# onolab-tmu/overiva

Measured on AMD Instinct MI355X. Metric: AuxIVA iterations/sec (2048 bins x 4000 frames x 8 mics), higher is better.
Workload: dtype f32

## Files before the change

overiva_amd/csrc/kernel_choice.h:

```cpp
#pragma once
#include <algorithm>
#include <functional>

#include "overiva_hip.h"

namespace oiva {

inline int ceil_div(int a, int b) { return (a + b - 1) / b; }
inline int round_up(int a, int b) { return (a + b - 1) / b * b; }

constexpr int kNarrowMax = 16;
constexpr int kWideMax = OIVA_MAX_CHANNELS;

constexpr int kBinsPerWave = 16;
constexpr int kPhasesPerWave = 4;
constexpr int kBlock = 256;
constexpr int kWaves = kBlock / 64;

enum class CovKind { Lane, Pair32, Pair64, Quad, Half16, Hmfma, Half16F64, Hmfma64, Mfma, Wide };
enum class PowKind { Lane, Mfma, Lds, Wide };
constexpr int kCovKinds = 10, kPowKinds = 4;
static_assert((int)CovKind::Wide + 1 == kCovKinds && (int)PowKind::Wide + 1 == kPowKinds, "one traits row per kind");

struct CovGeom {
// ... 74 lines not shown
    Partials partials;
    int launches;
    bool padded_x;
    bool quad_switch;
    bool fusable;
    bool update_arith;
    CovKind unit;
};
constexpr CovTraits kCovTraits[kCovKinds] = {
     {[](int M, int K) { return M >= 1 && M <= 8 && K >= 1 && K <= M; }, nullptr, kBinsPerWave, 16, Partials::F64, 1, false, false, true, false, CovKind::Lane},
     {[](int M, int K) { return M == 8 && K >= 3; }, [](int) { return 4; }, 32, 8, Partials::F64, 2, false, false, false, true, CovKind::Pair32},
     {[](int M, int) { return M == 8; }, [](int K) { return K >= 2 ? 2 : 1; }, 32, 8, Partials::F64, 2, false, false, false, false, CovKind::Pair64},
     {[](int M, int K) { return M >= 10 && M <= 16 && M % 2 == 0 && K >= 1 && K <= 4; }, [](int K) { return K >= 2 ? 2 : 1; }, kBinsPerWave, 8, Partials::F64, 2, true, true, false, true, CovKind::Quad},
     {[](int M, int K) { return M >= 10 && M <= 16 && M % 2 == 0 && K >= 1 && K <= 16; }, [](int K) { return K <= 8 ? 8 : (K <= 12 ? 12 : 16); }, 2, 16, Partials::F64, 2, true, true, false, true, CovKind::Half16},
     {[](int M, int K) { return M >= 10 && M <= 16 && M % 2 == 0 && K >= 9 && K <= 16; }, [](int K) { return K <= 8 ? 8 : (K <= 12 ? 12 : 16); }, 2, 32, Partials::F32IfPart32, 2, true, true, false, true, CovKind::Half16},
     {[](int M, int K) { return M >= 10 && M <= 16 && M % 2 == 0 && K >= 3 && K <= 16; }, [](int K) { return K <= 4 ? 4 : 8; }, 2, 16, Partials::F64, 2, true, true, false, true, CovKind::Mfma},
     {[](int M, int K) { return M == 16 && K >= 9 && K <= 16; }, [](int K) { return K <= 4 ? 4 : 8; }, 2, 32, Partials::F64, 2, true, true, false, true, CovKind::Mfma},
     {[](int M, int K) { return M >= 9 && M <= 16 && K >= 1 && K <= M; }, [](int) { return 1; }, kBinsPerWave, 4, Partials::Acc, 2, false, false, false, true, CovKind::Mfma},
     {[](int M, int K) { return M > kNarrowMax && M <= kWideMax && K >= 1 && K <= M; }, [](int K) { return std::min(K, 2); }, 1, 4, Partials::F64, 2, false, false, false, true, CovKind::Wide},
};
constexpr const CovTraits& traits(CovKind k) { return kCovTraits[(int)k]; }
constexpr bool partials_f64(const CovGeom& g, bool cov_f64) {
    return traits(g.kind).partials == Partials::F64 || (traits(g.kind).partials == Partials::Acc ? cov_f64 : !g.part32);
}

struct PowTraits {
    bool (*supported)(int M, int K);
    int (*sources)(int K);
    int bins;
    int quantum;
    bool padded_x;
    bool occupancy;
};
constexpr int pow_sources_per_pass(int , int K) {
    return K >= 3 ? 4 : (K >= 2 ? 2 : 1);
}
constexpr PowTraits kPowTraits[kPowKinds] = {
     {[](int M, int K) { return M >= 1 && M <= kNarrowMax && K >= 1 && K <= M && (M <= 8 || K <= 4); }, [](int K) { return pow_sources_per_pass(0, K); }, kBinsPerWave * kWaves, 4, false, true},
     {[](int M, int K) { return M > 8 && M <= kNarrowMax && K > 4 && K <= M; }, [](int K) { return pow_sources_per_pass(0, K); }, kBinsPerWave * kWaves, 4, true, false},
     {[](int M, int K) { return M == 16 && K > 4 && K <= M; }, [](int K) { return pow_sources_per_pass(0, K); }, kBinsPerWave * kWaves, 4, false, false},
     {[](int M, int K) { return M > kNarrowMax && M <= kWideMax && K >= 1 && K <= M; }, [](int K) { return K >= 3 ? 4 : K; }, kBinsPerWave * kWaves, 4, false, false},
};
constexpr const PowTraits& traits(PowKind k) { return kPowTraits[(int)k]; }

struct ChoiceIn {
    int T, F, F_total, M, K;
    int n_cu;
    bool cov_f64, upd_f64;
    bool cov_quad_on = true;
    bool cov_hmfma_on = true;
    bool part32 = false;
    bool kc_wide = true;
    bool power_lds = true;
};
struct Occupancy {
    std::function<int(int M, int kc, bool f64)> cov_blocks_per_cu;
    std::function<int(int M, int kp, int tcp)> pow_blocks_per_cu;
};

inline int lane_sources_per_pass(int M, int K, bool f64, bool short_axis, bool kc_wide) {
    const int regs = M * M * (f64 ? 2 : 1);
    int kc = 1;
    if (K >= 2 && regs * 2 <= 144) kc = 2;
    if (K >= 3 && regs * 4 <= 144) kc = 4;
    if (!f64 && kc_wide) {
        if (M == 7 && (K == 3 || K == 5 || K == 6 || (K == 7 && short_axis))) kc = 3;
        if (M == 5 && K >= 5) kc = 5;
    }
    return kc;
}

inline int pick_splits(int capacity, int blocks_per_split, int T, int min_frames) {
    int ns = std::max(1, capacity / std::max(1, blocks_per_split));
    ns = std::min(ns, std::max(1, T / std::max(1, min_frames)));
    return ns;
}

inline int mixed_min_splits(int capacity, int blocks_per_split, int T) {
    if (T >= 1024) return 8;
    const int one_round = std::max(1, capacity / std::max(1, blocks_per_split));
    return std::max(1, std::min(std::min(4, one_round), T / 16));
}

constexpr bool padded_channels(int M) { return M > 8 && M <= kNarrowMax && M % 2 == 1; }

inline CovKind choose_cov_kind(const ChoiceIn& c) {
    const int M = c.M, K = c.K;
    if (M > kNarrowMax) return CovKind::Wide;
    if (M <= 8) {
        if (!c.cov_f64 && traits(CovKind::Pair32).supported(M, K)) return CovKind::Pair32;
        if (c.cov_f64 && traits(CovKind::Pair64).supported(M, K)) return CovKind::Pair64;
        return CovKind::Lane;
    }
    const int Mc = M + (padded_channels(M) ? 1 : 0);
    if (!c.cov_f64 && c.cov_quad_on && traits(CovKind::Quad).supported(Mc, K) && (K <= 2 || c.upd_f64)) return CovKind::Quad;
    if (c.cov_quad_on && (c.cov_f64 ? traits(CovKind::Half16F64).supported(Mc, K) : K > 4 && traits(CovKind::Half16).supported(Mc, K))) {
        const CovKind hm = c.cov_f64 ? CovKind::Hmfma64 : CovKind::Hmfma;
        if (c.cov_hmfma_on && traits(hm).supported(Mc, K)) return hm;
        return c.cov_f64 ? CovKind::Half16F64 : CovKind::Half16;
    }
    return CovKind::Mfma;
}

inline CovGeom choose_cov(const ChoiceIn& c, const Occupancy& occ, int nsplit_req) {
    CovGeom g{};
    g.kind = choose_cov_kind(c);
// ... 18 lines not shown
                if (c.upd_f64) nsplit = std::max(nsplit, mixed_min_splits(n_cu * 2, blocks, T));
            }
            break;
        case CovKind::Half16:
        case CovKind::Hmfma:
        case CovKind::Half16F64:
        case CovKind::Hmfma64: {
            const bool hm = g.kind == CovKind::Hmfma || g.kind == CovKind::Hmfma64;
            if (nsplit <= 0) {
                const int chains = hm ? 8 : 4;
                nsplit = c.cov_f64 ? (!hm && g.kc == 4 && T >= 1024 ? 2 : 1) : ceil_div(T, chains * (c.upd_f64 ? 128 : 256));
                const int per_cu = hm ? (c.cov_f64 ? 2 : 3) : c.cov_f64 && g.kc == 4 ? 4 : 2;
                const int groups = hm ? F : g.nbg * ceil_div(K, g.kc);
                while (groups * nsplit < per_cu * n_cu && ceil_div(T, nsplit + 1) >= 64) ++nsplit;
            }
            if (t.partials == Partials::F32IfPart32) g.part32 = c.part32 ? 1 : 0;
            break;
        }
        case CovKind::Mfma:
            if (nsplit <= 0) {
                nsplit = ceil_div(T, 512);
                const int waves = F * ceil_div(K, 4);
                while (waves * nsplit < 2 * 4 * n_cu && ceil_div(T, nsplit + 1) >= 64) ++nsplit;
            }
            break;
        case CovKind::Lane:
        case CovKind::Pair32:
        case CovKind::Pair64:
            if (nsplit <= 0) {
                const int nz = ceil_div(K, g.kc);
                int bpc = 2;
                if (g.kind == CovKind::Lane && (bpc = occ.cov_blocks_per_cu(c.M, g.kc, c.cov_f64)) < 1) bpc = 2;
                nsplit = pick_splits(n_cu * bpc, g.nbg * nz, T, T >= 1024 ? 128 : 64);
                if (nsplit >= 12 && g.nbg * nz * nsplit >= n_cu * bpc) nsplit = nsplit * 7 / 8;
                const int cap = (g.nbg * nz * 32 >= n_cu) ? 32 : 64;
                nsplit = std::min(nsplit, cap);
                if (g.kind == CovKind::Pair32 && c.upd_f64) {
                    const int by_chain = T >= 1024 ? 8 : std::min(4, ceil_div(T, 256));
                    nsplit = std::max(nsplit, std::min(by_chain, mixed_min_splits(n_cu * bpc, g.nbg * nz, T)));
                }
            }
            break;
    }
    g.tc = round_up(ceil_div(T, nsplit), t.quantum);
    g.nsplit = ceil_div(T, g.tc);
    return g;
}

inline PowKind choose_pow_kind(const ChoiceIn& c) {
    if (c.M > kNarrowMax) return PowKind::Wide;
    if (!traits(PowKind::Mfma).supported(c.M, c.K)) return PowKind::Lane;
    if (c.power_lds && traits(PowKind::Lds).supported(c.M, c.K) && c.F >= kBinsPerWave * kWaves && c.T >= 16) return PowKind::Lds;
    return PowKind::Mfma;
}

inline PowGeom choose_pow(const ChoiceIn& c, const Occupancy& occ, int nsplit_req) {
    PowGeom g{};
    g.kind = choose_pow_kind(c);
    const PowTraits& t = traits(g.kind);
    const int T = c.T, n_cu = c.n_cu;
    g.nb = ceil_div(c.F, t.bins);
    g.kp = t.sources(c.K);
    int nsplit = nsplit_req;
    if (g.kind == PowKind::Wide) {
        const int groups = g.nb * ceil_div(c.K, g.kp);
        if (nsplit <= 0) nsplit = pick_splits(n_cu * 4, groups, T, 16);
        g.tcp = round_up(ceil_div(T, nsplit), t.quantum);
        g.nsplit = ceil_div(T, g.tcp);
        return g;
    }
    if (nsplit <= 0) {
        const int per_cu_x12 = (g.kp == 1 && c.M <= 8) ? 24 : 12;
        nsplit = pick_splits(std::max(n_cu / 2, n_cu * per_cu_x12 / std::max(c.M, 1)), g.nb, T, 32);
    }
    int tcp = round_up(ceil_div(T, nsplit), t.quantum);
    tcp = std::min(std::max(tcp, 4), kPowMaxFrames);
    g.tcp = tcp;
    g.nsplit = ceil_div(T, tcp);
    if (t.occupancy) {
        const int bpc = occ.pow_blocks_per_cu(c.M, g.kp, g.tcp);
        if (bpc > 0) g.rounds = (int)((((long long)g.nb * g.nsplit * ceil_div(c.K, g.kp)) + (long long)bpc * n_cu - 1) / ((long long)bpc * n_cu));
    }
    return g;
}

}
```

overiva_amd/csrc/kernels_cov.hip:

```cpp

#include <cstdint>
#include <cstdlib>

#include "oiva_device.h"
#include "cov_arith.h"

namespace oiva {
namespace {

constexpr int kCovUnroll = 2;
constexpr int kChunk = 16;
constexpr int kLdsStride = kBlock + 1;

template <int M, int KC, typename ACC, typename At>
__device__ __forceinline__ void reduce_and_store_at(At&& at, ACC* lds, double* __restrict__ Vpart, int F, int K, int k0) {
    constexpr int NA = M * M;
    constexpr int NACC = NA * KC;
    const int tid = threadIdx.x;
    const int bb = tid >> 4, aa = tid & 15;
    const int fo = blockIdx.x * kBinsPerWave + bb;
    double* out = Vpart + (((size_t)blockIdx.y * F + fo) * K + k0) * NA;
#pragma unroll
    for (int r0 = 0; r0 < NACC; r0 += kChunk) {
        __syncthreads();
// ... 56 lines not shown
    for (int kk = 0; kk < KC; ++kk)
#pragma unroll
        for (int a = 0; a < NA; ++a) acc[kk][a] = 0;

    const size_t frame_stride = (size_t)F * M;
    const float2* pbase = X + (size_t)fc * M;
    for (int i = 0; i < nsteps; i += kCovUnroll) {
        float xr[kCovUnroll][M], xi[kCovUnroll][M], rv[kCovUnroll][KC];
#pragma unroll
        for (int u = 0; u < kCovUnroll; ++u) {
            const int t = t_begin + q + 16 * (i + u);
            const int tcl = t < t_end ? t : T - 1;
            if constexpr (!UNIT) {
#pragma unroll
                for (int kk = 0; kk < KC; ++kk) {
                    const int k = k0 + kk;
                    rv[u][kk] = R[(size_t)tcl * K + (k < K ? k : K - 1)];
                }
            }
            load_x<M>(pbase + (size_t)tcl * frame_stride, xr[u], xi[u]);
        }
#pragma unroll
        for (int u = 0; u < kCovUnroll; ++u) {
            const int t = t_begin + q + 16 * (i + u);
            const bool live = t < t_end;
            ACC w[KC], ar[M], ai[M];
#pragma unroll
            for (int kk = 0; kk < KC; ++kk) {
                const bool on = live && (UNIT || k0 + kk < K);
                if constexpr (UNIT) {
                    w[kk] = on ? ACC(1) : ACC(0);
                } else if constexpr (sizeof(ACC) == 8) {
                    double rn = (double)rv[u][kk] * ginv[kk];
                    rn = rn < (double)kEpsR ? (double)kEpsR : rn;
                    w[kk] = on ? 1. / rn : 0.;
                } else {
                    w[kk] = on ? activation_weight(rv[u][kk], (float)ginv[kk]) : 0.f;
                }
            }
#pragma unroll
            for (int c = 0; c < M; ++c) {
                ar[c] = (ACC)xr[u][c];
                ai[c] = (ACC)xi[u][c];
            }
            accumulate<M, KC, UNIT, ACC>(acc, ar, ai, w);
        }
    }

    reduce_and_store<M, KC, ACC>(acc, lds, Vpart, F, K, k0);
}

constexpr int kDmaStages = 4;

template <int PIECES>
__device__ __forceinline__ void ring_read(unsigned addr, float4 (&v)[PIECES]);
template <int PIECES>
__device__ __forceinline__ void ring_read_rows(unsigned addr, float4 (&v)[PIECES]);

template <>
__device__ __forceinline__ void ring_read<4>(unsigned addr, float4 (&v)[4]) {
    asm volatile(
        "s_waitcnt vmcnt(12)\n\t"
        "ds_read_b128 %0, %4\n\t"
        "ds_read_b128 %1, %4 offset:1024\n\t"
        "ds_read_b128 %2, %4 offset:2048\n\t"
        "ds_read_b128 %3, %4 offset:3072\n\t"
        "s_waitcnt lgkmcnt(0)"
        : "=&v"(v[0]), "=&v"(v[1]), "=&v"(v[2]), "=&v"(v[3])
        : "v"(addr)
        : "memory");
}
template <>
__device__ __forceinline__ void ring_read<2>(unsigned addr, float4 (&v)[2]) {
    asm volatile(
        "s_waitcnt vmcnt(6)\n\t"
        "ds_read_b128 %0, %2\n\t"
        "ds_read_b128 %1, %2 offset:1024\n\t"
        "s_waitcnt lgkmcnt(0)"
        : "=&v"(v[0]), "=&v"(v[1])
        : "v"(addr)
        : "memory");
}

template <>
__device__ __forceinline__ void ring_read_rows<4>(unsigned addr, float4 (&v)[4]) {
    asm volatile(
        "s_waitcnt vmcnt(12)\n\t"
        "ds_read_b128 %0, %4\n\t"
        "ds_read_b128 %1, %4 offset:16\n\t"
        "ds_read_b128 %2, %4 offset:32\n\t"
        "ds_read_b128 %3, %4 offset:48\n\t"
        "s_waitcnt lgkmcnt(0)"
        : "=&v"(v[0]), "=&v"(v[1]), "=&v"(v[2]), "=&v"(v[3])
        : "v"(addr)
        : "memory");
}
template <>
__device__ __forceinline__ void ring_read_rows<2>(unsigned addr, float4 (&v)[2]) {
    asm volatile(
        "s_waitcnt vmcnt(6)\n\t"
        "ds_read_b128 %0, %2\n\t"
        "ds_read_b128 %1, %2 offset:16\n\t"
        "s_waitcnt lgkmcnt(0)"
        : "=&v"(v[0]), "=&v"(v[1])
        : "v"(addr)
        : "memory");
}

#ifdef OIVA_COVDMA_TRACE
__device__ long long g_cd_trace[8 * 2048];
#define CD_STAMP(slot)                                                                                                            \
    do {                                                                                                                          \
        if (threadIdx.x == 0 && blockIdx.z == 0) g_cd_trace[(blockIdx.y * gridDim.x + blockIdx.x) * 8 + (slot)] = wall_clock64(); \
    } while (0)
#else
#define CD_STAMP(slot) \
    do {               \
    } while (0)
#endif

template <int M, int KC>
__global__ __launch_bounds__(kBlock, 2) void cov_dma_kernel(const float2* __restrict__ X, const float* __restrict__ R,
                                                            float* __restrict__ wscale, int model, int raw,
                                                            double* __restrict__ Vpart, int T, int F, int K, int tc, int xplain) {
    constexpr int NA = M * M;
    constexpr int PIECES = M / 2;
    constexpr int STAGE = PIECES * 64;
    static_assert(M % 2 == 0 && (PIECES == 2 || PIECES == 4), "LDS-DMA path: M in {4, 8}");
    __shared__ float4 ring[kWaves * kDmaStages * STAGE];
    static_assert(sizeof(float4) * kWaves * kDmaStages * STAGE >= sizeof(float) * kChunk * kLdsStride,
                  "reduction scratch aliases the ring");

    const int tid = threadIdx.x;
    const int lane = tid & 63;
    const int wave = __builtin_amdgcn_readfirstlane(tid >> 6);
    const int b = lane & (kBinsPerWave - 1);
    const int ql = lane >> 4;
    const int q = wave * kPhasesPerWave + ql;
    const int f = blockIdx.x * kBinsPerWave + b;
    const int fc = f < F ? f : F - 1;
    const int k0 = blockIdx.z * KC;
    const int t_begin = blockIdx.y * tc;
    const int t_end = min(T, t_begin + tc);
    const int nsteps = (t_end - t_begin + 15) >> 4;

    constexpr bool kPacked = KC == 2;
    float acc[kPacked ? 1 : KC][kPacked ? 1 : NA];
    PkAcc2<M> pacc;
    if constexpr (kPacked) {
        pacc.clear();
    } else {
#pragma unroll
        for (int kk = 0; kk < KC; ++kk)
#pragma unroll
            for (int a = 0; a < NA; ++a) acc[kk][a] = 0.f;
    }

    float ginv[KC];
    float4* wring = ring + wave * kDmaStages * STAGE;
    const unsigned rd_base = (unsigned)(uintptr_t)(wring) + lane * 16;
    const size_t frame_stride = (size_t)F * M;
    const float2* pbase = X + (size_t)fc * M;
    using Rows = XRows<M>;
    const int row_off = Rows::offset(lane, blockIdx.x * kBinsPerWave, F);
    const unsigned rd_rows = (unsigned)(uintptr_t)(wring) + Rows::slot(b, ql) * 16;
    auto plain = [&](int i) { return M != 8 || x_group_plain(kXGroup * i, xplain); };

    auto issue = [&](int i, int s) {
        if (!plain(i)) {
            Rows::issue_nt(X, frame_stride, row_off, lane, t_begin + wave * kPhasesPerWave + 16 * i, i < nsteps ? t_end : 0, T, wring + s * STAGE);
            return;
        }
        const int t = t_begin + q + 16 * i;
        const int tcl = (i < nsteps && t < t_end) ? t : T - 1;
        const float2* src = pbase + (size_t)tcl * frame_stride;
#pragma unroll
        for (int j = 0; j < PIECES; ++j)
            __builtin_amdgcn_global_load_lds((gvoid_t*)(src + 2 * j), (lvoid_t*)(wring + s * STAGE + j * 64), 16, 0, 0);
    };
    const float m0 = ql == 0 ? 1.f : 0.f, m1 = ql == 1 ? 1.f : 0.f, m2 = ql == 2 ? 1.f : 0.f, m3 = ql == 3 ? 1.f : 0.f;
    auto consume = [&](int i, int s) {
        const int tw = min(t_begin + wave * kPhasesPerWave + 16 * i, T);
        const float* rp = R + (size_t)tw * K;
        float w[KC];
#pragma unroll
        for (int kk = 0; kk < KC; ++kk) {
            const int k = k0 + kk < K ? k0 + kk : K - 1;
            const float r = m0 * rp[k] + m1 * rp[K + k] + m2 * rp[2 * K + k] + m3 * rp[3 * K + k];
            const float live = (t_begin + wave * kPhasesPerWave + 16 * i + ql < t_end && k0 + kk < K) ? 1.f : 0.f;
            w[kk] = activation_weight(r, ginv[kk]) * live;
        }
        float4 v[PIECES];
        if (plain(i))
            ring_read<PIECES>(rd_base + s * STAGE * 16, v);
        else
            ring_read_rows<PIECES>(rd_rows + s * STAGE * 16, v);
#if defined(OIVA_COVDMA_ABLATE) && (OIVA_COVDMA_ABLATE & 1)
        if constexpr (kPacked) {
            if (v[0].x == 12345.f) pacc.add(reinterpret_cast<const v2f(&)[M]>(v), v2f{w[0], w[1]});
            return;
        }
#endif
        if constexpr (kPacked) {
            v2f x[M];
#pragma unroll
            for (int j = 0; j < PIECES; ++j) {
                x[2 * j] = v2f{v[j].x, v[j].y};
                x[2 * j + 1] = v2f{v[j].z, v[j].w};
            }
            pacc.add(x, v2f{w[0], w[1]});
        } else {
            float xr[M], xi[M];
#pragma unroll
            for (int j = 0; j < PIECES; ++j) {
                xr[2 * j] = v[j].x;
                xi[2 * j] = v[j].y;
                xr[2 * j + 1] = v[j].z;
                xi[2 * j + 1] = v[j].w;
            }
            accumulate<M, KC, false, float>(acc, xr, xi, w);
        }
    };

    CD_STAMP(0);
    issue(0, 0);
    issue(1, 1);
    issue(2, 2);
#pragma unroll
    for (int kk = 0; kk < KC; ++kk) {
        const int k = k0 + kk;
        ginv[kk] = 1.f;
        if (raw & 1) continue;
#if defined(OIVA_COVDMA_ABLATE) && (OIVA_COVDMA_ABLATE & 4)
        const float gamma = R[k < K ? k : K - 1] + 1.f;
#else
        const float gamma = (float)gamma_of(R, T, K, k < K ? k : K - 1);
#endif
        ginv[kk] = 1.f / gamma;
        if (blockIdx.x == 0 && blockIdx.y == 0 && threadIdx.x == 0 && k < K && wscale != nullptr)
            wscale[k] = model == OIVA_MODEL_LAPLACE ? gamma : sqrtf(gamma);
    }

    CD_STAMP(1);
    int i = 0;
    for (; i + 4 <= nsteps; i += 4) {
        issue(i + 3, 3); consume(i, 0);
        issue(i + 4, 0); consume(i + 1, 1);
        issue(i + 5, 1); consume(i + 2, 2);
        issue(i + 6, 2); consume(i + 3, 3);
// ... 144 lines not shown
```

overiva_amd/csrc/kernels_demix.hip:

```cpp
#include "oiva_device.h"
#include "demix_arith.h"

namespace oiva {
namespace {

constexpr int kPowUnroll = 2;

template <int M, int KP, bool NT = false>
__global__ __launch_bounds__(kBlock) void power_kernel(const float2* __restrict__ X, const float2* __restrict__ What,
                                                       float* __restrict__ Ppart, int T, int F, int K, int tcp, int rev, PowOrder ord,
                                                       int xplain, int xctc) {
    extern __shared__ __attribute__((aligned(16))) float sp[];
    const int tid = threadIdx.x;
    const int lane = tid & 63;
    const int wave = NT ? __builtin_amdgcn_readfirstlane(tid >> 6) : tid >> 6;
    const int b = lane & 15;
    const int q = lane >> 4;
    const int f = (blockIdx.x * kWaves + wave) * kBinsPerWave + b;
    const bool fvalid = f < F;
    const int fc = fvalid ? f : F - 1;
    const int k0 = blockIdx.z * KP;
    const int chunk = ord.cs > 0 ? power_chunk_tail_first(blockIdx.y, gridDim.y, ord) : (int)blockIdx.y;
    const int t_begin = chunk * tcp;
    const int t_end = min(T, t_begin + tcp);
    const int len = t_end - t_begin;
    const int nsteps = (len + 3) >> 2;
    const int ngroups = (nsteps + kPowUnroll - 1) / kPowUnroll;

    float wr[KP][M], wi[KP][M];
    load_wconj<M, KP>(What, fc, k0, K, wr, wi);

    const size_t frame_stride = (size_t)F * M;
    const float2* pbase = X + (size_t)fc * M;
    int off0 = 0, row_off = 0;
    float4* wrows = nullptr;
    if constexpr (NT) {
        __shared__ float4 rows[kWaves * kPowUnroll * 32 * M];
        off0 = t_begin % xctc;
        row_off = XRows<M>::offset(lane, (blockIdx.x * kWaves + wave) * kBinsPerWave, F);
        wrows = rows + wave * kPowUnroll * 32 * M;
    }
    for (int g = 0; g < ngroups; ++g) {
        const int i = (rev ? ngroups - 1 - g : g) * kPowUnroll;
        float xr[kPowUnroll][M], xi[kPowUnroll][M];
        bool plain[kPowUnroll];
#pragma unroll
        for (int u = 0; u < kPowUnroll; ++u) {
            const int tl = 4 * (i + u) + q;
            const int t = tl < len ? t_begin + tl : T - 1;
            plain[u] = !NT || x_group_plain(x_split_offset(off0, 4 * (i + u), xctc), xplain);
            if constexpr (NT) {
                if (!plain[u]) {
                    XRows<M>::issue_nt(X, frame_stride, row_off, lane, t_begin + 4 * (i + u), t_end, T, wrows + u * 32 * M);
                    continue;
                }
            }
            load_x<M>(pbase + (size_t)t * frame_stride, xr[u], xi[u]);
        }
#pragma unroll
        for (int u = 0; u < kPowUnroll; ++u) {
            const int tl = 4 * (i + u) + q;
            const bool live = tl < len;
            if constexpr (NT) {
                if (!plain[u]) {
                    const float4* v = wrows + u * 32 * M + XRows<M>::slot(b, q);
#pragma unroll
                    for (int j = 0; j < M / 2; ++j) {
                        const float4 p = v[j];
                        xr[u][2 * j] = p.x, xi[u][2 * j] = p.y, xr[u][2 * j + 1] = p.z, xi[u][2 * j + 1] = p.w;
                    }
                }
            }
#pragma unroll
            for (int kk = 0; kk < KP; ++kk) {
                float yr, yi;
                demix_one<M>(wr[kk], wi[kk], xr[u], xi[u], yr, yi);
                float pw = fmaf(yr, yr, yi * yi);
                pw = fvalid ? pw : 0.f;
                pw = row16_sum(pw);
                if (b == 0 && live) sp[(wave * tcp + tl) * KP + kk] = pw;
            }
        }
    }
    __syncthreads();
    for (int e = tid; e < len * KP; e += kBlock) {
        const int tl = e / KP, kk = e - tl * KP;
        float s = sp[(0 * tcp + tl) * KP + kk];
#pragma unroll
        for (int w = 1; w < kWaves; ++w) s += sp[(w * tcp + tl) * KP + kk];
        if (k0 + kk < K) Ppart[((size_t)blockIdx.x * T + t_begin + tl) * K + k0 + kk] = s;
    }
}

template <int M, int KP>
__global__ __launch_bounds__(kBlock) void stats_kernel(const float2* __restrict__ X, const float2* __restrict__ What,
                                                       float* __restrict__ Spart, int T, int F, int K, int tc) {
    __shared__ float lds[3 * KP * (kBlock + 1)];
    const int tid = threadIdx.x;
    const int b = tid & 15;
    const int q = tid >> 4;
    const int f = blockIdx.x * kBinsPerWave + b;
    const int fc = f < F ? f : F - 1;
    const int k0 = blockIdx.z * KP;
    const int t_begin = blockIdx.y * tc;
    const int t_end = min(T, t_begin + tc);
    const int nsteps = (t_end - t_begin + 15) >> 4;

    float wr[KP][M], wi[KP][M];
    load_wconj<M, KP>(What, fc, k0, K, wr, wi);
    float nr[KP], ni[KP], dn[KP];
#pragma unroll
    for (int kk = 0; kk < KP; ++kk) nr[kk] = ni[kk] = dn[kk] = 0.f;

    const size_t frame_stride = (size_t)F * M;
    const float2* px = X + ((size_t)(t_begin + q) * F + fc) * M;
    for (int i = 0; i < nsteps; ++i) {
        const int t = t_begin + q + 16 * i;
        if (t < t_end) {
            float xr[M], xi[M];
            load_x<M>(px, xr, xi);
#pragma unroll
            for (int kk = 0; kk < KP; ++kk) {
                float yr, yi;
                demix_one<M>(wr[kk], wi[kk], xr, xi, yr, yi);
                nr[kk] = fmaf(xr[0], yr, fmaf(xi[0], yi, nr[kk]));
                ni[kk] = fmaf(xr[0], yi, fmaf(-xi[0], yr, ni[kk]));
                dn[kk] = fmaf(yr, yr, fmaf(yi, yi, dn[kk]));
            }
        }
        px += 16 * frame_stride;
    }
#pragma unroll
    for (int kk = 0; kk < KP; ++kk) {
// ... 175 lines not shown
```

overiva_amd/csrc/oiva_device.h:

```cpp
#pragma once
#include "oiva_internal.h"

#include <type_traits>
#include <utility>

namespace oiva {

constexpr float kEpsR = 1e-15f;

__device__ __forceinline__ double block_sum(double v, double* scratch) {
#pragma unroll
    for (int off = 32; off > 0; off >>= 1) v += __shfl_xor(v, off, 64);
    const int wave = threadIdx.x >> 6;
    __syncthreads();
    if ((threadIdx.x & 63) == 0) scratch[wave] = v;
    __syncthreads();
    double s = 0.;
#pragma unroll
    for (int w = 0; w < kWaves; ++w) s += scratch[w];
    return s;
}

__device__ __forceinline__ double gamma_of(const float* __restrict__ R, int T, int K, int k) {
    const double* S = reinterpret_cast<const double*>(R + rsum_offset_floats(T, K));
    const int nblk = rsum_blocks(T);
    double s = 0.;
    for (int b = 0; b < nblk; ++b) s += S[(size_t)b * K + k];
    return s / (double)T;
}

__device__ __forceinline__ float activation_weight(float r, float ginv) {
    float rn = r * ginv;
    rn = rn < kEpsR ? kEpsR : rn;
    return 1.f / rn;
}

template <int M>
__device__ __forceinline__ void load_x(const float2* __restrict__ p, float (&xr)[M], float (&xi)[M]) {
    if constexpr (M % 2 == 0) {
        const float4* p4 = reinterpret_cast<const float4*>(p);
#pragma unroll
        for (int i = 0; i < M / 2; ++i) {
            const float4 v = p4[i];
            xr[2 * i] = v.x;
            xi[2 * i] = v.y;
            xr[2 * i + 1] = v.z;
            xi[2 * i + 1] = v.w;
        }
    } else {
#pragma unroll
        for (int i = 0; i < M; ++i) {
            const float2 v = p[i];
            xr[i] = v.x;
            xi[i] = v.y;
        }
    }
}

typedef __attribute__((address_space(1))) const void gvoid_t;
typedef __attribute__((address_space(3))) void lvoid_t;
template <int M>
struct XRows {
    static_assert(M == 4 || M == 8, "whole 1-KB instructions of 16-byte pieces");
    static constexpr int kPieces = M / 2;
    static constexpr int kLanesPerRow = 16 * kPieces;
    static constexpr int kFramesPerInstr = 64 / kLanesPerRow;
    static __device__ __forceinline__ int frame(int lane, int j) { return j * kFramesPerInstr + lane / kLanesPerRow; }
    static __device__ __forceinline__ int offset(int lane, int f0, int F) {
        const int r = lane % kLanesPerRow, f = f0 + r / kPieces;
        return (f < F ? f : F - 1) * M + (r % kPieces) * 2;
    }
    static __device__ __forceinline__ int slot(int b, int q) { return (q * 16 + b) * kPieces; }
    static __device__ __forceinline__ void issue_nt(const float2* __restrict__ X, size_t frame_stride, int off, int lane, int t0, int t_lim,
                                                    int T, float4* stage) {
#pragma unroll
        for (int j = 0; j < kPieces; ++j) {
            const int t = t0 + frame(lane, j);
            const float2* src = X + (size_t)(t < t_lim ? t : T - 1) * frame_stride + off;
            __builtin_amdgcn_global_load_lds((gvoid_t*)src, (lvoid_t*)(stage + j * 64), 16, 0,  2);
        }
    }
};

using f32x4 = __attribute__((ext_vector_type(4))) float;
using f64x4 = __attribute__((ext_vector_type(4))) double;

template <typename REAL>
struct Mfma;
template <>
struct Mfma<float> {
    using acc_t = f32x4;
    static __device__ __forceinline__ acc_t run(float a, float b, acc_t c) {
        return __builtin_amdgcn_mfma_f32_16x16x4f32(a, b, c, 0, 0, 0);
    }
    static __device__ __forceinline__ int row(int lane, int r) { return (lane >> 4) * 4 + r; }
};
template <>
struct Mfma<double> {
    using acc_t = f64x4;
    static __device__ __forceinline__ acc_t run(double a, double b, acc_t c) {
        return __builtin_amdgcn_mfma_f64_16x16x4f64(a, b, c, 0, 0, 0);
    }
    static __device__ __forceinline__ int row(int lane, int r) { return (lane >> 4) + 4 * r; }
};

template <int CTRL>
__device__ __forceinline__ int dpp32(int x) {
    return __builtin_amdgcn_update_dpp(0, x, CTRL, 0xF, 0xF, true);
}
template <int CTRL>
__device__ __forceinline__ float dpp(float v) { return __int_as_float(dpp32<CTRL>(__float_as_int(v))); }
template <int CTRL>
__device__ __forceinline__ unsigned dpp(unsigned v) { return (unsigned)dpp32<CTRL>((int)v); }
template <int CTRL>
__device__ __forceinline__ double dpp(double v) {
    return __hiloint2double(dpp32<CTRL>(__double2hiint(v)), dpp32<CTRL>(__double2loint(v)));
}
template <int CTRL, int BANKS>
__device__ __forceinline__ int dpp32_banks(int old, int x) {
    return __builtin_amdgcn_update_dpp(old, x, CTRL, 0xF, BANKS, false);
}
template <int CTRL, int BANKS>
__device__ __forceinline__ float dpp_banks(float old, float v) {
    return __int_as_float(dpp32_banks<CTRL, BANKS>(__float_as_int(old), __float_as_int(v)));
}
template <int CTRL, int BANKS>
__device__ __forceinline__ double dpp_banks(double old, double v) {
    return __hiloint2double(dpp32_banks<CTRL, BANKS>(__double2hiint(old), __double2hiint(v)),
                            dpp32_banks<CTRL, BANKS>(__double2loint(old), __double2loint(v)));
}
template <typename F, int... I>
__device__ __forceinline__ void static_for_impl(F&& f, std::integer_sequence<int, I...>) {
    (f(std::integral_constant<int, I>{}), ...);
}
template <int N, typename F>
// ... 38 lines not shown
```

overiva_amd/csrc/plan.hip:

```cpp
#include <algorithm>
#include <cmath>
#include <cstdint>
#include <cstdlib>
#include <cstring>
#include <mutex>
#include <string>
#include <vector>

#include "host_io.h"
#include "host_util.h"
#include "oiva_internal.h"
#include "resident.h"

using namespace oiva;

namespace {

constexpr int kGraphBatch = 8;
constexpr int kGraphMaxIters = 32;
constexpr int kGraphCache = 6;

}

struct oiva_plan {
    int device = 0;
    int T = 0, F = 0, M = 0, K = 0, model = 0, F_total = 0;
    HandleStream stream;
    DeviceArena mem;

    const float2* X = nullptr;
    float2* X_owned = nullptr;
    float2* X_pad = nullptr;
    float2* What = nullptr;
    double2* What64 = nullptr;
    bool what64_valid = false;
    double* Cx = nullptr;
    void* Vpart = nullptr;
    float* Ppart = nullptr;
    int ppart_alloc = 0;
    float* Plocal = nullptr;
    void* Wwide = nullptr;
    float* R = nullptr;
    float* wscale = nullptr;
    float* Spart = nullptr;
    float2* Y = nullptr;
    double2* scratch_c = nullptr;
    double* scratch_p = nullptr;

    CovGeom cov{};
    bool cov_quad_on = true;
    bool cov_hmfma_on = true;
    bool fuse_cov_update = false;
    int power_reverse = 1;
    double x_resident_mb = kXResidentDefaultMB;
    CovGeom stg{};
    PowGeom pw{};
    int n_cu = 256;
    int vpart_splits_alloc = 0;

    bool have_x = false, have_cx = false, have_w = false;
    bool pad_valid = false;
    bool wscale_pending = false;
    int raw_weights = 0;
    int prec = 0;
    bool upd_f64() const { return prec & OIVA_PREC_UPDATE_F64; }
    bool cov_f64() const { return prec & OIVA_PREC_COV_F64; }
    bool vpart_f64() const { return partials_f64(cov, cov_f64()); }
    int use_graph = 0;
    OgiveState og{};
    bool og_ready = false;
    int og_mode = 0, og_model = 0;
    hipGraphExec_t og_graph = nullptr;
    int og_graph_n = 0, og_graph_phase = -1;
    double og_graph_mu = 0., og_graph_tol = 0.;
    ResidentGeom rg{};
    bool res_ok = false;
    bool res_on = false;
    void* res_block = nullptr;
    float* res_parts = nullptr;
    float* res_psum = nullptr;
    double* res_vpart = nullptr;
    double* res_rsum = nullptr;
    float2* res_wpub = nullptr;
    unsigned* res_flags = nullptr;
    float2* res_what = nullptr;
    double2* res_what64 = nullptr;
    unsigned* res_code_host = nullptr;
    unsigned long long* res_stamps = nullptr;
    size_t res_block_bytes = 0;
    unsigned res_epoch = 0;
    int res_last_code = 0, res_launches = 0, res_fallbacks = 0, res_stamped = 0;
    int res_timeout_ms = 0, res_stall = -1, res_stall_iter = 0;
    char* res_loop_buf = nullptr;
    bool res_loopback = false;
    bool res_trace = false;
    unsigned long long* res_trace_buf = nullptr;
    int res_trace_iters = 0;
    char* res_gath[OIVA_XCHG_MAX_RANKS] = {};
    int res_rank = 0, res_world = 1;
    bool fx_on = false, fx_loopback = false;
    char* fx_gath[OIVA_XCHG_MAX_RANKS] = {};
    int fx_rank = 0, fx_world = 1;
    int fx_nblk_own = 1, fx_nblk_peer = 1;
    char* fx_loop_buf = nullptr;
    unsigned* fx_state = nullptr;
    unsigned* fx_flag_host = nullptr;
    int fx_timeout_ms = 0, fx_stall = 0;
    HandleStream io_stream;
    double2* io_c128[kHostRingSlots] = {};
    size_t io_c128_bytes = 0;
    size_t io_slab_bytes = 0;
    float2* ck_what = nullptr;
    double2* ck_what64 = nullptr;
    bool ck_valid = false, ck_what64_valid = false;
    GraphCache graphs{kGraphCache};
};

namespace {

ChoiceIn choice_in(const oiva_plan* p) {
    static const bool kc_wide = [] { const char* v = std::getenv("OIVA_COV_KC_WIDE"); return !(v && v[0] == '0'); }();
    static const bool power_lds = [] { const char* v = std::getenv("OIVA_POWER_LDS"); return !(v && v[0] == '0'); }();
    const char* pv = std::getenv("OIVA_HMFMA_PART32");
    ChoiceIn c{};
    c.T = p->T, c.F = p->F, c.F_total = p->F_total, c.M = p->M, c.K = p->K, c.n_cu = p->n_cu;
    c.cov_f64 = p->cov_f64(), c.upd_f64 = p->upd_f64();
    c.cov_quad_on = p->cov_quad_on, c.cov_hmfma_on = p->cov_hmfma_on;
    c.part32 = pv && pv[0] == '1';
    c.kc_wide = kc_wide, c.power_lds = power_lds;
    return c;
}
Occupancy device_occupancy(int* asked = nullptr) {
    Occupancy o;
    o.cov_blocks_per_cu = [asked](int M, int kc, bool f64) {
        int n = 0;
        if (cov_blocks_per_cu(M, kc, f64, &n) != hipSuccess) n = 0;
        if (asked) asked[0] = n;
        return n;
    };
    o.pow_blocks_per_cu = [asked](int M, int kp, int tcp) {
        int n = 0;
        if (pow_blocks_per_cu(M, kp, tcp, &n) != hipSuccess) n = 0;
        if (asked) asked[1] = n;
        return n;
    };
    return o;
}
void choose_cov_geom(oiva_plan* p, int nsplit_req) { p->cov = choose_cov(choice_in(p), device_occupancy(), nsplit_req); }
void choose_pow_geom(oiva_plan* p, int nsplit_req) { p->pw = choose_pow(choice_in(p), device_occupancy(), nsplit_req); }

void choose_stats_geom(oiva_plan* p) {
    CovGeom g;
    if (p->M > kNarrowMax) {
        g.nbg = ceil_div(p->F_total, 64);
        g.kc = 2;
        const int nsplit = std::min(16, pick_splits(p->n_cu * 4, g.nbg * ceil_div(p->K, g.kc), p->T, 128));
        g.tc = round_up(ceil_div(p->T, nsplit), 16);
        g.nsplit = ceil_div(p->T, g.tc);
        p->stg = g;
        return;
    }
    p->stg = stats_geom(p->T, p->F, p->K, p->n_cu);
}

int drop_graph(oiva_plan* p) {
    const int rc = p->graphs.clear();
    if (rc) return rc;
    if (p->og_graph) {
        OIVA_TRY_HIP(hipGraphExecDestroy(p->og_graph));
        p->og_graph = nullptr;
    }
    return OIVA_OK;
}

size_t vpart_floats(const oiva_plan* p, int nsplit) { return (size_t)nsplit * p->F * p->K * p->M * p->M; }

int ensure_vpart(oiva_plan* p) {
    if (p->cov.nsplit > p->vpart_splits_alloc) {
        p->mem.release(&p->Vpart);
        OIVA_TRY_HIP(p->mem.take_one(&p->Vpart, (vpart_floats(p, p->cov.nsplit) + 2) * sizeof(double)));
        p->vpart_splits_alloc = p->cov.nsplit;
    }
    return OIVA_OK;
}

XPolicy x_policy(const oiva_plan* p) { return choose_x_policy(p->x_resident_mb, p->T, p->F, p->M, p->cov_f64(), p->cov, p->pw); }
CovGeom cov_geom_now(const oiva_plan* p) {
    CovGeom g = p->cov;
    g.xplain = x_policy(p).xplain();
    return g;
}

int stage_power(oiva_plan* p) {
    PowGeom g = p->pw;
    g.xplain = x_policy(p).xplain();
    g.xctc = p->cov.tc;
    if (p->power_reverse) {
        g.rev = 1;
        if (g.rounds > 1 || p->power_reverse > 1) g.ord = make_pow_order(g.nsplit, g.tcp, p->cov.nsplit, p->cov.tc);
    }
    OIVA_TRY_HIP(launch_power(p->stream, p->X, p->X_pad && p->pad_valid ? p->X_pad : nullptr, p->What, p->Ppart, p->T, p->F, p->M, p->K, g));
    return OIVA_OK;
// ... 885 lines not shown
}

int oiva_plan_get_cov_splits(oiva_plan* p, int* nsplit) {
    OIVA_NEED(p && nsplit, OIVA_ERR_ARG, "null argument");
    *nsplit = p->cov.nsplit;
    return OIVA_OK;
}

int oiva_plan_set_cov_splits(oiva_plan* p, int nsplit) {
    OIVA_NEED(p, OIVA_ERR_ARG, "null plan");
    OIVA_NEED(nsplit >= 0 && nsplit <= p->T, OIVA_ERR_ARG, "bad split count");
    return change_geometry(p, [&] { choose_cov_geom(p, nsplit); return OIVA_OK; });
}

int oiva_plan_set_cov_quad(oiva_plan* p, int enable, int* active) {
    OIVA_NEED(p, OIVA_ERR_ARG, "null plan");
    return change_geometry(p, [&] {
        p->cov_quad_on = enable != 0;
        choose_cov_geom(p, 0);
        if (active) *active = traits(p->cov.kind).quad_switch;
        return OIVA_OK;
    });
}

int oiva_plan_set_fuse_cov_update(oiva_plan* p, int enable, int* active) {
    OIVA_NEED(p, OIVA_ERR_ARG, "null plan");
    if (enable >= 0) {
        const int rc = change_geometry(p, [&] { p->fuse_cov_update = enable != 0; return OIVA_OK; });
        if (rc) return rc;
    }
    if (active) *active = cov_update_applies(p) ? 1 : 0;
    return OIVA_OK;
}

int oiva_plan_set_cov_hmfma(oiva_plan* p, int enable) {
    OIVA_NEED(p, OIVA_ERR_ARG, "null plan");
    return change_geometry(p, [&] { p->cov_hmfma_on = enable != 0; choose_cov_geom(p, 0); return OIVA_OK; });
}

int oiva_plan_set_pow_splits(oiva_plan* p, int nsplit) {
    OIVA_NEED(p, OIVA_ERR_ARG, "null plan");
    OIVA_NEED(nsplit >= 0 && nsplit <= p->T, OIVA_ERR_ARG, "bad split count");
    return change_geometry(p, [&] { choose_pow_geom(p, nsplit); return OIVA_OK; });
}

int oiva_plan_set_power_reverse(oiva_plan* p, int enable) {
    OIVA_NEED(p, OIVA_ERR_ARG, "null plan");
    return change_geometry(p, [&] { p->power_reverse = enable < 0 ? 0 : enable > 2 ? 2 : enable; return OIVA_OK; });
}

int oiva_plan_set_x_resident_mb(oiva_plan* p, double mb) {
    OIVA_NEED(p, OIVA_ERR_ARG, "null plan");
    OIVA_NEED(mb == mb, OIVA_ERR_ARG, "the budget is not a number");
    return change_geometry(p, [&] { p->x_resident_mb = mb; return OIVA_OK; });
}

int oiva_plan_get_x_resident(oiva_plan* p, int* n16, int* nt, int* reason) {
    OIVA_NEED(p && n16 && nt && reason, OIVA_ERR_ARG, "null argument");
    const XPolicy x = x_policy(p);
    *n16 = x.n16, *nt = x.nt ? 1 : 0, *reason = (int)x.why;
    return OIVA_OK;
}

int oiva_plan_use_graph(oiva_plan* p, int enable) {
    OIVA_NEED(p, OIVA_ERR_ARG, "null plan");
    DeviceGuard guard(p->device);
    p->use_graph = enable ? 1 : 0;
    if (!enable) return drop_graph(p);
    if (p->have_x && p->have_cx && p->have_w && (p->F == p->F_total || p->fx_on)) return build_graphs(p);
    return OIVA_OK;
}

int oiva_plan_set_precision(oiva_plan* p, int flags) {
    OIVA_NEED(p, OIVA_ERR_ARG, "null plan");
    OIVA_NEED((flags & ~(OIVA_PREC_UPDATE_F64 | OIVA_PREC_UPDATE_ROWS | OIVA_PREC_COV_F64)) == 0, OIVA_ERR_ARG, "unknown precision flag");
    return change_geometry(p, [&] {
        if ((flags & OIVA_PREC_UPDATE_F64) && p->have_w && !p->what64_valid) {
            std::vector<double2> wh;
            int rc;
            if ((rc = download_what(p, wh)) || (rc = upload_what(p, wh))) return rc;
        }
        const bool cov_changed = ((flags ^ p->prec) & (OIVA_PREC_COV_F64 | (traits(p->cov.kind).update_arith ? OIVA_PREC_UPDATE_F64 : 0))) != 0;
        p->prec = flags;
        if (cov_changed) choose_cov_geom(p, 0);
        return (int)OIVA_OK;
    });
}

int oiva_plan_set_resident(oiva_plan* p, int enable) {
    OIVA_NEED(p, OIVA_ERR_ARG, "null plan");
    if (!enable) {
        p->res_on = false;
        return OIVA_OK;
    }
    OIVA_NEED(p->res_ok, OIVA_ERR_ARG,
              "shape does not qualify for the X-resident iteration (4 or 8 channels, 1 or 2 sources with background channels, "
              "16 bins x <= 256 frames per compute unit)");
    DeviceGuard guard(p->device);
    int rc = resident_alloc(p);
    if (rc) return rc;
    p->res_on = true;
    return OIVA_OK;
}

int oiva_plan_set_resident_splits(oiva_plan* p, int nsplit) {
    OIVA_NEED(p && nsplit >= 0, OIVA_ERR_ARG, "bad arguments");
    OIVA_NEED(!p->res_on, OIVA_ERR_STATE, "switch the resident iteration off before changing its geometry");
    DeviceGuard guard(p->device);
    ResidentGeom g;
    const bool ok = resident_geometry(p->T, p->F, p->M, p->K, p->n_cu, nsplit, &g);
    OIVA_NEED(ok || nsplit == 0, OIVA_ERR_ARG, "the shape does not fit on chip with that many frame splits");
    if (p->res_block) {
        OIVA_TRY_HIP(hipStreamSynchronize(p->stream));
        p->mem.release(&p->res_block);
    }
    p->res_ok = ok;
    if (ok) p->rg = g;
    return OIVA_OK;
}

int oiva_plan_resident_loopback(oiva_plan* p, int world) {
    OIVA_NEED(p, OIVA_ERR_ARG, "null plan");
    OIVA_NEED(world >= 0 && world <= OIVA_XCHG_MAX_RANKS, OIVA_ERR_ARG, "bad number of ranks");
    OIVA_NEED(!p->res_on, OIVA_ERR_STATE, "switch the resident iteration off before changing its exchange");
    DeviceGuard guard(p->device);
    if (p->res_loop_buf) {
        OIVA_TRY_HIP(hipStreamSynchronize(p->stream));
        p->mem.release(&p->res_loop_buf);
    }
    p->res_loopback = false;
    p->res_world = 1;
    p->res_rank = 0;
    for (auto& g : p->res_gath) g = nullptr;
    if (world <= 1) return OIVA_OK;
    OIVA_NEED(p->res_ok, OIVA_ERR_ARG, "shape does not qualify for the X-resident iteration");
    OIVA_NEED(p->F == p->F_total, OIVA_ERR_STATE, "loop-back plays the other ranks with zeros: the plan must own all bins");
    const size_t bytes = (size_t)2 * world * p->rg.NS * p->rg.TW * p->K * sizeof(float);
// ... 407 lines not shown
```

Measured before the change: 5457.

## Double-buffer streamed X reads in power kernel and resize its split when streaming

When X is streamed rather than held resident, the power kernel now stages every frame group through a two-stage LDS ring filled by global_load_lds. It overlaps the next group's load with demixing the current one, and writes power values through explicit ds_write. The ring_read helpers move into a shared header and take the number of loads left in flight as a parameter, so the covariance kernel and the power kernel can share them. The split chooser also picks about one block per CU for the lane power kernel with two sources when X is streamed, and the plan re-derives the power geometry when the residency budget or precision changes. The changes add LDS pressure and hand-written waitcnt logic, and the smaller grid may lower latency hiding.

```diff
diff --git a/overiva_amd/csrc/kernel_choice.h b/overiva_amd/csrc/kernel_choice.h
--- a/overiva_amd/csrc/kernel_choice.h
+++ b/overiva_amd/csrc/kernel_choice.h
@@ -150,6 +150,7 @@
     bool part32 = false;
     bool kc_wide = true;
     bool power_lds = true;
+    double x_resident_mb = 0.;
 };
 struct Occupancy {
     std::function<int(int M, int kc, bool f64)> cov_blocks_per_cu;
@@ -274,6 +275,14 @@
     if (!traits(PowKind::Mfma).supported(c.M, c.K)) return PowKind::Lane;
     if (c.power_lds && traits(PowKind::Lds).supported(c.M, c.K) && c.F >= kBinsPerWave * kWaves && c.T >= 16) return PowKind::Lds;
     return PowKind::Mfma;
+}
+
+inline bool x_streams_by_kernels(const ChoiceIn& c, PowKind pk) {
+    CovGeom cg{};
+    cg.kind = choose_cov_kind(c), cg.tc = kXGroup;
+    PowGeom pg{};
+    pg.kind = pk, pg.tcp = 4;
+    return choose_x_policy(c.x_resident_mb, c.T, c.F, c.M, c.cov_f64, cg, pg).nt;
 }
 
 inline PowGeom choose_pow(const ChoiceIn& c, const Occupancy& occ, int nsplit_req) {
@@ -294,6 +303,12 @@
     if (nsplit <= 0) {
         const int per_cu_x12 = (g.kp == 1 && c.M <= 8) ? 24 : 12;
         nsplit = pick_splits(std::max(n_cu / 2, n_cu * per_cu_x12 / std::max(c.M, 1)), g.nb, T, 32);
+        if (g.kind == PowKind::Lane && g.kp == 2 && x_streams_by_kernels(c, g.kind)) {
+            const int one = pick_splits(n_cu, g.nb, T, 32);
+            const int tcp1 = std::min(std::max(round_up(ceil_div(T, one), t.quantum), 4), kPowMaxFrames);
+            const long long grid = (long long)g.nb * ceil_div(T, tcp1);
+            if (grid <= n_cu && grid * 8 >= (long long)n_cu * 7) nsplit = one;
+        }
     }
     int tcp = round_up(ceil_div(T, nsplit), t.quantum);
     tcp = std::min(std::max(tcp, 4), kPowMaxFrames);
diff --git a/overiva_amd/csrc/kernels_cov.hip b/overiva_amd/csrc/kernels_cov.hip
--- a/overiva_amd/csrc/kernels_cov.hip
+++ b/overiva_amd/csrc/kernels_cov.hip
@@ -132,61 +132,6 @@
 
 constexpr int kDmaStages = 4;
 
-template <int PIECES>
-__device__ __forceinline__ void ring_read(unsigned addr, float4 (&v)[PIECES]);
-template <int PIECES>
-__device__ __forceinline__ void ring_read_rows(unsigned addr, float4 (&v)[PIECES]);
-
-template <>
-__device__ __forceinline__ void ring_read<4>(unsigned addr, float4 (&v)[4]) {
-    asm volatile(
-        "s_waitcnt vmcnt(12)\n\t"
-        "ds_read_b128 %0, %4\n\t"
-        "ds_read_b128 %1, %4 offset:1024\n\t"
-        "ds_read_b128 %2, %4 offset:2048\n\t"
-        "ds_read_b128 %3, %4 offset:3072\n\t"
-        "s_waitcnt lgkmcnt(0)"
-        : "=&v"(v[0]), "=&v"(v[1]), "=&v"(v[2]), "=&v"(v[3])
-        : "v"(addr)
-        : "memory");
-}
-template <>
-__device__ __forceinline__ void ring_read<2>(unsigned addr, float4 (&v)[2]) {
-    asm volatile(
-        "s_waitcnt vmcnt(6)\n\t"
-        "ds_read_b128 %0, %2\n\t"
-        "ds_read_b128 %1, %2 offset:1024\n\t"
-        "s_waitcnt lgkmcnt(0)"
-        : "=&v"(v[0]), "=&v"(v[1])
-        : "v"(addr)
-        : "memory");
-}
-
-template <>
-__device__ __forceinline__ void ring_read_rows<4>(unsigned addr, float4 (&v)[4]) {
-    asm volatile(
-        "s_waitcnt vmcnt(12)\n\t"
-        "ds_read_b128 %0, %4\n\t"
-        "ds_read_b128 %1, %4 offset:16\n\t"
-        "ds_read_b128 %2, %4 offset:32\n\t"
-        "ds_read_b128 %3, %4 offset:48\n\t"
-        "s_waitcnt lgkmcnt(0)"
-        : "=&v"(v[0]), "=&v"(v[1]), "=&v"(v[2]), "=&v"(v[3])
-        : "v"(addr)
-        : "memory");
-}
-template <>
-__device__ __forceinline__ void ring_read_rows<2>(unsigned addr, float4 (&v)[2]) {
-    asm volatile(
-        "s_waitcnt vmcnt(6)\n\t"
-        "ds_read_b128 %0, %2\n\t"
-        "ds_read_b128 %1, %2 offset:16\n\t"
-        "s_waitcnt lgkmcnt(0)"
-        : "=&v"(v[0]), "=&v"(v[1])
-        : "v"(addr)
-        : "memory");
-}
-
 #ifdef OIVA_COVDMA_TRACE
 __device__ long long g_cd_trace[8 * 2048];
 #define CD_STAMP(slot)                                                                                                            \
@@ -272,9 +217,9 @@
         }
         float4 v[PIECES];
         if (plain(i))
-            ring_read<PIECES>(rd_base + s * STAGE * 16, v);
+            ring_read<PIECES, (kDmaStages - 1) * PIECES>(rd_base + s * STAGE * 16, v);
         else
-            ring_read_rows<PIECES>(rd_rows + s * STAGE * 16, v);
+            ring_read_rows<PIECES, (kDmaStages - 1) * PIECES>(rd_rows + s * STAGE * 16, v);
 #if defined(OIVA_COVDMA_ABLATE) && (OIVA_COVDMA_ABLATE & 1)
         if constexpr (kPacked) {
             if (v[0].x == 12345.f) pacc.add(reinterpret_cast<const v2f(&)[M]>(v), v2f{w[0], w[1]});
diff --git a/overiva_amd/csrc/kernels_demix.hip b/overiva_amd/csrc/kernels_demix.hip
--- a/overiva_amd/csrc/kernels_demix.hip
+++ b/overiva_amd/csrc/kernels_demix.hip
@@ -5,6 +5,12 @@
 namespace {
 
 constexpr int kPowUnroll = 2;
+constexpr int kPowStages = 2;
+
+__device__ __forceinline__ void lds_store(float* base, int idx, float v) {
+    asm volatile("ds_write_b32 %0, %1" : : "v"((unsigned)(uintptr_t)base + 4u * (unsigned)idx), "v"(v) : "memory");
+}
+__device__ __forceinline__ void lds_stores_done() { asm volatile("s_waitcnt vmcnt(0) lgkmcnt(0)" ::: "memory"); }
 
 template <int M, int KP, bool NT = false>
 __global__ __launch_bounds__(kBlock) void power_kernel(const float2* __restrict__ X, const float2* __restrict__ What,
@@ -25,60 +31,82 @@
     const int t_end = min(T, t_begin + tcp);
     const int len = t_end - t_begin;
     const int nsteps = (len + 3) >> 2;
-    const int ngroups = (nsteps + kPowUnroll - 1) / kPowUnroll;
+    [[maybe_unused]] const int ngroups = (nsteps + kPowUnroll - 1) / kPowUnroll;
 
     float wr[KP][M], wi[KP][M];
     load_wconj<M, KP>(What, fc, k0, K, wr, wi);
 
     const size_t frame_stride = (size_t)F * M;
-    const float2* pbase = X + (size_t)fc * M;
-    int off0 = 0, row_off = 0;
-    float4* wrows = nullptr;
+    [[maybe_unused]] const float2* pbase = X + (size_t)fc * M;
     if constexpr (NT) {
-        __shared__ float4 rows[kWaves * kPowUnroll * 32 * M];
-        off0 = t_begin % xctc;
-        row_off = XRows<M>::offset(lane, (blockIdx.x * kWaves + wave) * kBinsPerWave, F);
-        wrows = rows + wave * kPowUnroll * 32 * M;
-    }
-    for (int g = 0; g < ngroups; ++g) {
-        const int i = (rev ? ngroups - 1 - g : g) * kPowUnroll;
-        float xr[kPowUnroll][M], xi[kPowUnroll][M];
-        bool plain[kPowUnroll];
-#pragma unroll
-        for (int u = 0; u < kPowUnroll; ++u) {
-            const int tl = 4 * (i + u) + q;
-            const int t = tl < len ? t_begin + tl : T - 1;
-            plain[u] = !NT || x_group_plain(x_split_offset(off0, 4 * (i + u), xctc), xplain);
-            if constexpr (NT) {
-                if (!plain[u]) {
-                    XRows<M>::issue_nt(X, frame_stride, row_off, lane, t_begin + 4 * (i + u), t_end, T, wrows + u * 32 * M);
-                    continue;
-                }
-            }
-            load_x<M>(pbase + (size_t)t * frame_stride, xr[u], xi[u]);
-        }
-#pragma unroll
-        for (int u = 0; u < kPowUnroll; ++u) {
-            const int tl = 4 * (i + u) + q;
-            const bool live = tl < len;
-            if constexpr (NT) {
-                if (!plain[u]) {
-                    const float4* v = wrows + u * 32 * M + XRows<M>::slot(b, q);
-#pragma unroll
-                    for (int j = 0; j < M / 2; ++j) {
-                        const float4 p = v[j];
-                        xr[u][2 * j] = p.x, xi[u][2 * j] = p.y, xr[u][2 * j + 1] = p.z, xi[u][2 * j + 1] = p.w;
-                    }
-                }
-            }
+        constexpr int PIECES = XRows<M>::kPieces, STAGE = PIECES * 64;
+        __shared__ float4 ring[kWaves * kPowStages * STAGE];
+        float4* wring = ring + wave * kPowStages * STAGE;
+        const int off0 = t_begin % xctc;
+        const int row_off = XRows<M>::offset(lane, (blockIdx.x * kWaves + wave) * kBinsPerWave, F);
+        const unsigned rd_rows = (unsigned)(uintptr_t)wring + XRows<M>::slot(b, q) * 16;
+        auto step_of = [&](int n) { return rev ? nsteps - 1 - n : n; };
+        auto issue = [&](int n, int s) {
+            const int i = n < nsteps ? step_of(n) : 0;
+            const int t_lim = n < nsteps ? t_end : 0;
+            if (x_group_plain(x_split_offset(off0, 4 * i, xctc), xplain))
+                XRows<M>::template issue<0>(X, frame_stride, row_off, lane, t_begin + 4 * i, t_lim, T, wring + s * STAGE);
+            else
+                XRows<M>::template issue<2>(X, frame_stride, row_off, lane, t_begin + 4 * i, t_lim, T, wring + s * STAGE);
+        };
+        auto consume = [&](int n, int s) {
+            float4 v[PIECES];
+            ring_read_rows<PIECES, (kPowStages - 1) * PIECES>(rd_rows + s * STAGE * 16, v);
+            float xr[M], xi[M];
+#pragma unroll
+            for (int j = 0; j < PIECES; ++j) xr[2 * j] = v[j].x, xi[2 * j] = v[j].y, xr[2 * j + 1] = v[j].z, xi[2 * j + 1] = v[j].w;
+            const int tl = 4 * step_of(n) + q;
 #pragma unroll
             for (int kk = 0; kk < KP; ++kk) {
                 float yr, yi;
-                demix_one<M>(wr[kk], wi[kk], xr[u], xi[u], yr, yi);
+                demix_one<M>(wr[kk], wi[kk], xr, xi, yr, yi);
                 float pw = fmaf(yr, yr, yi * yi);
                 pw = fvalid ? pw : 0.f;
                 pw = row16_sum(pw);
-                if (b == 0 && live) sp[(wave * tcp + tl) * KP + kk] = pw;
+                if (b == 0 && tl < len) lds_store(sp, (wave * tcp + tl) * KP + kk, pw);
+            }
+        };
+        static_assert(kPowStages == 2, "the loop is unrolled over the stages by hand");
+#pragma unroll
+        for (int kk = 0; kk < KP; ++kk)
+#pragma unroll
+            for (int m = 0; m < M; ++m) asm volatile("" : "+v"(wr[kk][m]), "+v"(wi[kk][m]));
+        issue(0, 0);
+        int n = 0;
+        for (; n + 2 <= nsteps; n += 2) {
+            issue(n + 1, 1); consume(n, 0);
+            issue(n + 2, 0); consume(n + 1, 1);
+        }
+        if (n < nsteps) { issue(n + 1, 1); consume(n, 0); }
+        lds_stores_done();
+    } else {
+        for (int g = 0; g < ngroups; ++g) {
+            const int i = (rev ? ngroups - 1 - g : g) * kPowUnroll;
+            float xr[kPowUnroll][M], xi[kPowUnroll][M];
+#pragma unroll
+            for (int u = 0; u < kPowUnroll; ++u) {
+                const int tl = 4 * (i + u) + q;
+                const int t = tl < len ? t_begin + tl : T - 1;
+                load_x<M>(pbase + (size_t)t * frame_stride, xr[u], xi[u]);
+            }
+#pragma unroll
+            for (int u = 0; u < kPowUnroll; ++u) {
+                const int tl = 4 * (i + u) + q;
+                const bool live = tl < len;
+#pragma unroll
+                for (int kk = 0; kk < KP; ++kk) {
+                    float yr, yi;
+                    demix_one<M>(wr[kk], wi[kk], xr[u], xi[u], yr, yi);
+                    float pw = fmaf(yr, yr, yi * yi);
+                    pw = fvalid ? pw : 0.f;
+                    pw = row16_sum(pw);
+                    if (b == 0 && live) sp[(wave * tcp + tl) * KP + kk] = pw;
+                }
             }
         }
     }
diff --git a/overiva_amd/csrc/oiva_device.h b/overiva_amd/csrc/oiva_device.h
--- a/overiva_amd/csrc/oiva_device.h
+++ b/overiva_amd/csrc/oiva_device.h
@@ -71,16 +71,70 @@
         return (f < F ? f : F - 1) * M + (r % kPieces) * 2;
     }
     static __device__ __forceinline__ int slot(int b, int q) { return (q * 16 + b) * kPieces; }
-    static __device__ __forceinline__ void issue_nt(const float2* __restrict__ X, size_t frame_stride, int off, int lane, int t0, int t_lim,
-                                                    int T, float4* stage) {
+    template <int AUX>
+    static __device__ __forceinline__ void issue(const float2* __restrict__ X, size_t frame_stride, int off, int lane, int t0, int t_lim, int T,
+                                                 float4* stage) {
 #pragma unroll
         for (int j = 0; j < kPieces; ++j) {
             const int t = t0 + frame(lane, j);
             const float2* src = X + (size_t)(t < t_lim ? t : T - 1) * frame_stride + off;
-            __builtin_amdgcn_global_load_lds((gvoid_t*)src, (lvoid_t*)(stage + j * 64), 16, 0,  2);
+            __builtin_amdgcn_global_load_lds((gvoid_t*)src, (lvoid_t*)(stage + j * 64), 16, 0, AUX);
         }
     }
+    static __device__ __forceinline__ void issue_nt(const float2* __restrict__ X, size_t frame_stride, int off, int lane, int t0, int t_lim,
+                                                    int T, float4* stage) {
+        issue<2>(X, frame_stride, off, lane, t0, t_lim, T, stage);
+    }
 };
+
+template <int PIECES, int INFLIGHT>
+__device__ __forceinline__ void ring_read(unsigned addr, float4 (&v)[PIECES]) {
+    static_assert(PIECES == 2 || PIECES == 4, "M in {4, 8}");
+    if constexpr (PIECES == 4)
+        asm volatile(
+            "s_waitcnt vmcnt(%5)\n\t"
+            "ds_read_b128 %0, %4\n\t"
+            "ds_read_b128 %1, %4 offset:1024\n\t"
+            "ds_read_b128 %2, %4 offset:2048\n\t"
+            "ds_read_b128 %3, %4 offset:3072\n\t"
+            "s_waitcnt lgkmcnt(0)"
+            : "=&v"(v[0]), "=&v"(v[1]), "=&v"(v[2]), "=&v"(v[3])
+            : "v"(addr), "n"(INFLIGHT)
+            : "memory");
+    else
+        asm volatile(
+            "s_waitcnt vmcnt(%3)\n\t"
+            "ds_read_b128 %0, %2\n\t"
+            "ds_read_b128 %1, %2 offset:1024\n\t"
+            "s_waitcnt lgkmcnt(0)"
+            : "=&v"(v[0]), "=&v"(v[1])
+            : "v"(addr), "n"(INFLIGHT)
+            : "memory");
+}
+template <int PIECES, int INFLIGHT>
+__device__ __forceinline__ void ring_read_rows(unsigned addr, float4 (&v)[PIECES]) {
+    static_assert(PIECES == 2 || PIECES == 4, "M in {4, 8}");
+    if constexpr (PIECES == 4)
+        asm volatile(
+            "s_waitcnt vmcnt(%5)\n\t"
+            "ds_read_b128 %0, %4\n\t"
+            "ds_read_b128 %1, %4 offset:16\n\t"
+            "ds_read_b128 %2, %4 offset:32\n\t"
+            "ds_read_b128 %3, %4 offset:48\n\t"
+            "s_waitcnt lgkmcnt(0)"
+            : "=&v"(v[0]), "=&v"(v[1]), "=&v"(v[2]), "=&v"(v[3])
+            : "v"(addr), "n"(INFLIGHT)
+            : "memory");
+    else
+        asm volatile(
+            "s_waitcnt vmcnt(%3)\n\t"
+            "ds_read_b128 %0, %2\n\t"
+            "ds_read_b128 %1, %2 offset:16\n\t"
+            "s_waitcnt lgkmcnt(0)"
+            : "=&v"(v[0]), "=&v"(v[1])
+            : "v"(addr), "n"(INFLIGHT)
+            : "memory");
+}
 
 using f32x4 = __attribute__((ext_vector_type(4))) float;
 using f64x4 = __attribute__((ext_vector_type(4))) double;
diff --git a/overiva_amd/csrc/plan.hip b/overiva_amd/csrc/plan.hip
--- a/overiva_amd/csrc/plan.hip
+++ b/overiva_amd/csrc/plan.hip
@@ -52,6 +52,7 @@
     bool cov_hmfma_on = true;
     bool fuse_cov_update = false;
     int power_reverse = 1;
+    int pow_splits_req = 0;
     double x_resident_mb = kXResidentDefaultMB;
     CovGeom stg{};
     PowGeom pw{};
@@ -128,6 +129,7 @@
     c.cov_quad_on = p->cov_quad_on, c.cov_hmfma_on = p->cov_hmfma_on;
     c.part32 = pv && pv[0] == '1';
     c.kc_wide = kc_wide, c.power_lds = power_lds;
+    c.x_resident_mb = p->x_resident_mb;
     return c;
 }
 Occupancy device_occupancy(int* asked = nullptr) {
@@ -147,7 +149,10 @@
     return o;
 }
 void choose_cov_geom(oiva_plan* p, int nsplit_req) { p->cov = choose_cov(choice_in(p), device_occupancy(), nsplit_req); }
-void choose_pow_geom(oiva_plan* p, int nsplit_req) { p->pw = choose_pow(choice_in(p), device_occupancy(), nsplit_req); }
+void choose_pow_geom(oiva_plan* p, int nsplit_req) {
+    p->pow_splits_req = nsplit_req;
+    p->pw = choose_pow(choice_in(p), device_occupancy(), nsplit_req);
+}
 
 void choose_stats_geom(oiva_plan* p) {
     CovGeom g;
@@ -1139,7 +1144,7 @@
 int oiva_plan_set_x_resident_mb(oiva_plan* p, double mb) {
     OIVA_NEED(p, OIVA_ERR_ARG, "null plan");
     OIVA_NEED(mb == mb, OIVA_ERR_ARG, "the budget is not a number");
-    return change_geometry(p, [&] { p->x_resident_mb = mb; return OIVA_OK; });
+    return change_geometry(p, [&] { p->x_resident_mb = mb; choose_pow_geom(p, p->pow_splits_req); return OIVA_OK; });
 }
 
 int oiva_plan_get_x_resident(oiva_plan* p, int* n16, int* nt, int* reason) {
@@ -1170,6 +1175,7 @@
         const bool cov_changed = ((flags ^ p->prec) & (OIVA_PREC_COV_F64 | (traits(p->cov.kind).update_arith ? OIVA_PREC_UPDATE_F64 : 0))) != 0;
         p->prec = flags;
         if (cov_changed) choose_cov_geom(p, 0);
+        if (cov_changed) choose_pow_geom(p, p->pow_splits_req);
         return (int)OIVA_OK;
     });
 }
```

Measured after the change: 5651, median of 6. +3.5%, better.
